# lnkloveating/MediQuery-RAG

Measured on AMD Instinct MI355X. Metric: queries/s (embed+top-k, k=5, b=256) over 1M×768 corpus; p50 single-query ms, higher is better.
Workload: dtype f32 (exact 3-way bf16 split, fp32 accumulate; exact fp32 top-k)

## Files before the change

mediquery-rag_amd/csrc/gemm_epi.hpp:

```cpp
#pragma once

#include "gemm_f32.hpp"
#include "gemm_x6p.hpp"

namespace mq {

enum Epi {
  EPI_BIAS = 0,
  EPI_GELU_ERF = 1,
  EPI_GELU_TANH = 2,
  EPI_RESID = 3,
  EPI_RESID_STATS = 4,
  EPI_RESID_LN_STATS = 5,
  EPI_BIAS_LNFOLD = 6,
  EPI_GELU_ERF_LNFOLD = 7,
  EPI_GELU_TANH_LNFOLD = 8
};
constexpr bool epi_is_lnfold(int epi) { return epi >= EPI_BIAS_LNFOLD && epi <= EPI_GELU_TANH_LNFOLD; }

__device__ __forceinline__ float gelu_erf(float x) {
  const float z = fabsf(x) * 0.70710678118654752f;
  const float t = __builtin_amdgcn_rcpf(fmaf(0.5f, z, 1.0f));
  float p = 0.17087277f;
  p = fmaf(p, t, -0.82215223f);
  p = fmaf(p, t, 1.48851587f);
  p = fmaf(p, t, -1.13520398f);
  p = fmaf(p, t, 0.27886807f);
  p = fmaf(p, t, -0.18628806f);
  p = fmaf(p, t, 0.09678418f);
  p = fmaf(p, t, 0.37409196f);
  p = fmaf(p, t, 1.00002368f);
  p = fmaf(p, t, -1.26551223f);
  const float e = t * __builtin_amdgcn_exp2f(fmaf(-z, z, p) * 1.4426950408889634f);
  return x * (x >= 0.f ? fmaf(-0.5f, e, 1.0f) : 0.5f * e);
}
__device__ __forceinline__ float gelu_tanh(float x) {
  const float u = 0.7978845608028654f * fmaf(0.044715f * x, x * x, x);
  return x * __builtin_amdgcn_rcpf(1.0f + __builtin_amdgcn_exp2f(u * -2.8853900817779268f));
}

template <int EPI>
__device__ __forceinline__ float epi_apply(float v) {
  if constexpr (EPI == EPI_GELU_ERF || EPI == EPI_GELU_ERF_LNFOLD) return gelu_erf(v);
  if constexpr (EPI == EPI_GELU_TANH || EPI == EPI_GELU_TANH_LNFOLD) return gelu_tanh(v);
  return v;
}

__device__ __forceinline__ void ln_merge(const floatx4 (&p)[kLnMaxParts / 2], float eps, float& mean, float& rstd) {
  float sum = 0.f;
#pragma unroll
  for (int i = 0; i < kLnMaxParts / 2; ++i) {
    sum += p[i].x;
    sum += p[i].z;
  }
  mean = sum * (1.0f / (float)kLnMaxParts);
  float m2 = 0.f;
#pragma unroll
  for (int i = 0; i < kLnMaxParts / 2; ++i) {
    const float d0 = p[i].x - mean, d1 = p[i].z - mean;
    m2 = __fmaf_rn((float)kLnPartW * d0, d0, m2 + p[i].y);
    m2 = __fmaf_rn((float)kLnPartW * d1, d1, m2 + p[i].w);
  }
  rstd = 1.0f / sqrtf(__fmaf_rn(m2, 1.0f / (float)(kLnPartW * kLnMaxParts), eps));
}
template <int MB>
__device__ __forceinline__ void ln_row_own(const float* __restrict__ stats, int wr0, int M, float eps, int lane,
                                           float& mean, float& rstd) {
  const int c = lane & 15;
  const int row = min(wr0 + 16 * min(c >> 2, MB - 1) + 4 * (lane >> 4) + (c & 3), M - 1);
  const floatx4* src = reinterpret_cast<const floatx4*>(stats + (int64_t)row * (2 * kLnMaxParts));
  floatx4 p[kLnMaxParts / 2];
#pragma unroll
  for (int i = 0; i < kLnMaxParts / 2; ++i) p[i] = src[i];
  ln_merge(p, eps, mean, rstd);
}
__device__ __forceinline__ float ln_row_bcast(float v, int lane, int m, int e) {
  return __shfl(v, (lane & 48) + 4 * m + e);
}
__device__ __forceinline__ float row16_sum(float v) {
  v += __int_as_float(__builtin_amdgcn_update_dpp(0, __float_as_int(v), 0xB1, 0xF, 0xF, false));
  v += __int_as_float(__builtin_amdgcn_update_dpp(0, __float_as_int(v), 0x4E, 0xF, 0xF, false));
  v += __int_as_float(__builtin_amdgcn_update_dpp(0, __float_as_int(v), 0x141, 0xF, 0xF, false));
  v += __int_as_float(__builtin_amdgcn_update_dpp(0, __float_as_int(v), 0x140, 0xF, 0xF, false));
  return v;
}

template <int EPI, int TM, int TN>
__device__ __forceinline__ void store_wave_tile(floatx16 (&acc)[TM][TN], int wr0, int wc0, int M, int N,
                                                const float* __restrict__ bias, const float* __restrict__ resid,
                                                int ldr, float* __restrict__ out, int ldo, int lane) {
  if (wr0 + TM * 32 <= M && wc0 + TN * 32 <= N) {
    float bv[TN];
#pragma unroll
    for (int tn = 0; tn < TN; ++tn) bv[tn] = bias[wc0 + tn * 32 + (lane & 31)];
    float rv[TM][TN][16];
    if constexpr (EPI == EPI_RESID) {
      const __amdgpu_buffer_rsrc_t rr = __builtin_amdgcn_make_buffer_rsrc(
          (void*)(resid + (int64_t)wr0 * ldr + wc0), (short)0, 0x7fffffff, 0x00020000);
      const int rl = (4 * (lane >> 5) * ldr + (lane & 31)) * 4;
#pragma unroll
      for (int tm = 0; tm < TM; ++tm)
#pragma unroll
        for (int tn = 0; tn < TN; ++tn)
#pragma unroll
          for (int e = 0; e < 16; ++e)
            rv[tm][tn][e] = __uint_as_float(
                __builtin_amdgcn_raw_buffer_load_b32(rr, rl, (acc_row(tm, e, 0) * ldr + tn * 32) * 4, 0));
    }
    const __amdgpu_buffer_rsrc_t ro = __builtin_amdgcn_make_buffer_rsrc(
        (void*)(out + (int64_t)wr0 * ldo + wc0), (short)0, 0x7fffffff, 0x00020000);
    const int ol = (4 * (lane >> 5) * ldo + (lane & 31)) * 4;
#pragma unroll
    for (int tm = 0; tm < TM; ++tm)
#pragma unroll
      for (int tn = 0; tn < TN; ++tn)
#pragma unroll
        for (int e = 0; e < 16; ++e) {
          float v = epi_apply<EPI>(acc[tm][tn][e] + bv[tn]);
          if constexpr (EPI == EPI_RESID) v += rv[tm][tn][e];
          __builtin_amdgcn_raw_buffer_store_b32(__float_as_uint(v), ro, ol, (acc_row(tm, e, 0) * ldo + tn * 32) * 4, 0);
        }
    return;
  }
#pragma unroll
  for (int tn = 0; tn < TN; ++tn) {
    const int col = wc0 + tn * 32 + (lane & 31);
    if (col >= N) continue;
    const float b = bias[col];
#pragma unroll
    for (int tm = 0; tm < TM; ++tm)
#pragma unroll
      for (int e = 0; e < 16; ++e) {
        const int row = wr0 + acc_row(tm, e, lane);
        if (row >= M) continue;
        float v = epi_apply<EPI>(acc[tm][tn][e] + b);
        if constexpr (EPI == EPI_RESID) v += resid[(int64_t)row * ldr + col];
        out[(int64_t)row * ldo + col] = v;
      }
  }
}

typedef unsigned uint2v_t __attribute__((ext_vector_type(2)));
template <int ER, int MB, int NB>
__device__ __forceinline__ void store_wave_tile16_ln_stats(floatx4 (&acc)[MB][NB], int wr0, int wc0, int M,
                                                           const float* __restrict__ bias,
                                                           const float* __restrict__ resid, int ldr,
                                                           float* __restrict__ out, int ldo, int lane,
                                                           const LnFold& lf) {
  static_assert(NB * 16 == kLnPartW && MB <= 4, "partials are per kLnPartW-column wave tile");
  const int c = lane & 15, g = lane >> 4;
  const bool ln_r = lf.stats_in != nullptr;
  float own_mu = 0.f, own_rho = 1.0f;
  if (ln_r) ln_row_own<MB>(lf.stats_in, wr0, M, lf.eps, lane, own_mu, own_rho);
  float gv[NB];
#pragma unroll
  for (int n = 0; n < NB; ++n) {
    const int col = wc0 + n * 16 + c;
    const float bb = bias[col] + (ln_r ? lf.b[col] : 0.f);
    gv[n] = ln_r ? lf.g[col] : 1.0f;
#pragma unroll
    for (int m = 0; m < MB; ++m)
#pragma unroll
      for (int e = 0; e < 4; ++e) acc[m][n][e] += bb;
  }
  const __amdgpu_buffer_rsrc_t rr =
      __builtin_amdgcn_make_buffer_rsrc((void*)(resid + wc0), (short)0, 0x7fffffff, 0x00020000);
  const __amdgpu_buffer_rsrc_t ro =
      __builtin_amdgcn_make_buffer_rsrc((void*)(out + wc0), (short)0, 0x7fffffff, 0x00020000);
  const __amdgpu_buffer_rsrc_t rs = __builtin_amdgcn_make_buffer_rsrc(
      (void*)(lf.stats_out + 2 * (wc0 / kLnPartW)), (short)0, 0x7fffffff, 0x00020000);
#pragma unroll
  for (int m = 0; m < MB; ++m)
#pragma unroll
    for (int eh = 0; eh < 4; eh += ER) {
      float v[ER][NB];
#pragma unroll
      for (int e2 = 0; e2 < ER; ++e2) {
        const int lo = (min(wr0 + m * 16 + 4 * g + eh + e2, M - 1) * ldr + c) * 4;
#pragma unroll
        for (int n = 0; n < NB; ++n)
          v[e2][n] = __uint_as_float(__builtin_amdgcn_raw_buffer_load_b32(rr, lo, n * 64, 0));
      }
#pragma unroll
      for (int e2 = 0; e2 < ER; ++e2) {
        const int e = eh + e2, row = wr0 + m * 16 + 4 * g + e;
        const float mu = ln_row_bcast(own_mu, lane, m, e), rho = ln_row_bcast(own_rho, lane, m, e);
        const int so = (row * ldo + c) * 4;
        float sum = 0.f;
#pragma unroll
        for (int n = 0; n < NB; ++n) {
          v[e2][n] = __fmaf_rn((v[e2][n] - mu) * rho, gv[n], acc[m][n][e]);
          sum += v[e2][n];
          if (row < M) __builtin_amdgcn_raw_buffer_store_b32(__float_as_uint(v[e2][n]), ro, so, n * 64, 0);
        }
        const float mean = row16_sum(sum) * (1.0f / (float)kLnPartW);
        float m2 = 0.f;
#pragma unroll
        for (int n = 0; n < NB; ++n) {
          const float d = v[e2][n] - mean;
          m2 = __fmaf_rn(d, d, m2);
        }
        m2 = row16_sum(m2);
        if (c == 0 && row < M) {
          uint2v_t pr;
          pr.x = __float_as_uint(mean);
          pr.y = __float_as_uint(m2);
          __builtin_amdgcn_raw_buffer_store_b64(pr, rs, row * (kLnMaxParts * 8), 0, 0);
        }
      }
    }
}

template <int EPI, int MB, int NB>
__device__ __forceinline__ void store_wave_tile16(floatx4 (&acc)[MB][NB], int wr0, int wc0, int M, int N,
                                                  const float* __restrict__ bias, const float* __restrict__ resid,
                                                  int ldr, float* __restrict__ out, int ldo, int lane,
                                                  const LnFold& lf = LnFold{}) {
  const int c = lane & 15, g = lane >> 4;
  if constexpr (EPI == EPI_RESID_LN_STATS) {
    store_wave_tile16_ln_stats<1>(acc, wr0, wc0, M, bias, resid, ldr, out, ldo, lane, lf);
    return;
  }
  constexpr bool FOLD = epi_is_lnfold(EPI);
  static_assert(!FOLD || MB <= 4, "one lane of a 16-lane row group per row of the wave tile");
  float own_mu = 0.f, own_rho = 0.f;
  if constexpr (FOLD) ln_row_own<MB>(lf.stats_in, wr0, M, lf.eps, lane, own_mu, own_rho);
  if (wr0 + MB * 16 <= M && wc0 + NB * 16 <= N) {
    float bv[NB], sv[NB];
#pragma unroll
    for (int n = 0; n < NB; ++n) bv[n] = bias[wc0 + n * 16 + c];
    if constexpr (FOLD) {
#pragma unroll
      for (int n = 0; n < NB; ++n) sv[n] = lf.s[wc0 + n * 16 + c];
    }
    const __amdgpu_buffer_rsrc_t rr = __builtin_amdgcn_make_buffer_rsrc(
        (void*)(resid + (EPI == EPI_RESID ? (int64_t)wr0 * ldr + wc0 : 0)), (short)0, 0x7fffffff, 0x00020000);
    const int rl = (4 * g * ldr + c) * 4;
    const __amdgpu_buffer_rsrc_t ro = __builtin_amdgcn_make_buffer_rsrc(
        (void*)(out + (int64_t)wr0 * ldo + wc0), (short)0, 0x7fffffff, 0x00020000);
    const int ol = (4 * g * ldo + c) * 4;
#pragma unroll
    for (int m = 0; m < MB; ++m) {
      float rv[NB][4];
      if constexpr (EPI == EPI_RESID) {
#pragma unroll
        for (int n = 0; n < NB; ++n)
#pragma unroll
          for (int e = 0; e < 4; ++e)
            rv[n][e] = __uint_as_float(
                __builtin_amdgcn_raw_buffer_load_b32(rr, rl, ((m * 16 + e) * ldr + n * 16) * 4, 0));
      }
      if constexpr (FOLD) {
#pragma unroll
        for (int e = 0; e < 4; ++e) {
          const float mu = ln_row_bcast(own_mu, lane, m, e), rho = ln_row_bcast(own_rho, lane, m, e);
#pragma unroll
          for (int n = 0; n < NB; ++n) {
            const float v = epi_apply<EPI>(__fmaf_rn(rho, __fmaf_rn(-mu, sv[n], acc[m][n][e]), bv[n]));
            __builtin_amdgcn_raw_buffer_store_b32(__float_as_uint(v), ro, ol, ((m * 16 + e) * ldo + n * 16) * 4, 0);
          }
        }
      } else {
#pragma unroll
        for (int n = 0; n < NB; ++n)
#pragma unroll
          for (int e = 0; e < 4; ++e) {
            float v = epi_apply<EPI>(acc[m][n][e] + bv[n]);
            if constexpr (EPI == EPI_RESID) v += rv[n][e];
            __builtin_amdgcn_raw_buffer_store_b32(__float_as_uint(v), ro, ol, ((m * 16 + e) * ldo + n * 16) * 4, 0);
          }
      }
    }
    return;
  }
  if constexpr (FOLD) {
#pragma unroll
    for (int m = 0; m < MB; ++m) {
      float mu[4], rho[4];
#pragma unroll
      for (int e = 0; e < 4; ++e) {
        mu[e] = ln_row_bcast(own_mu, lane, m, e);
        rho[e] = ln_row_bcast(own_rho, lane, m, e);
      }
#pragma unroll
      for (int n = 0; n < NB; ++n) {
        const int col = wc0 + n * 16 + c;
        if (col < N) {
          const float b = bias[col], sn = lf.s[col];
#pragma unroll
          for (int e = 0; e < 4; ++e) {
            const int row = wr0 + m * 16 + 4 * g + e;
            if (row < M)
              out[(int64_t)row * ldo + col] = epi_apply<EPI>(__fmaf_rn(rho[e], __fmaf_rn(-mu[e], sn, acc[m][n][e]), b));
          }
        }
      }
    }
    return;
  }
#pragma unroll
  for (int n = 0; n < NB; ++n) {
    const int col = wc0 + n * 16 + c;
    if (col >= N) continue;
    const float b = bias[col];
#pragma unroll
    for (int m = 0; m < MB; ++m)
#pragma unroll
      for (int e = 0; e < 4; ++e) {
        const int row = wr0 + m * 16 + 4 * g + e;
        if (row >= M) continue;
        float v = epi_apply<EPI>(acc[m][n][e] + b);
        if constexpr (EPI == EPI_RESID) v += resid[(int64_t)row * ldr + col];
        out[(int64_t)row * ldo + col] = v;
      }
  }
}

}
```

mediquery-rag_amd/csrc/gemm_x6p.hip:

```cpp
#include <algorithm>

#include "gemm_epi.hpp"
#include "gemm_x6p.hpp"

namespace mq {
namespace {

typedef __attribute__((address_space(3))) void x6p_lds_t;

__device__ __forceinline__ void x6p_glds(const void* base, unsigned voff, unsigned lds_dst) {
  const uint64_t b64 = (uint64_t)(uintptr_t)base;
  base = (const void*)(uintptr_t)(((uint64_t)__builtin_amdgcn_readfirstlane((unsigned)(b64 >> 32)) << 32) |
                                  (unsigned)__builtin_amdgcn_readfirstlane((unsigned)b64));
  unsigned keep;
  asm volatile("s_mov_b32 %0, m0\n\ts_mov_b32 m0, %3\n\ts_nop 0\n\tglobal_load_lds_dwordx4 %1, %2\n\ts_mov_b32 m0, %0"
               : "=&s"(keep)
               : "v"(voff), "s"(base), "s"(__builtin_amdgcn_readfirstlane(lds_dst))
               : "memory");
}

__device__ __forceinline__ int a_swz(int q) { return q ^ (q >> 1); }

typedef __bf16 bf16x2_t __attribute__((ext_vector_type(2)));
typedef float float2_t __attribute__((ext_vector_type(2)));
__device__ __forceinline__ unsigned cvt_pk_bf16(float lo, float hi) {
  float2_t v;
  v.x = lo;
  v.y = hi;
  return __builtin_bit_cast(unsigned, __builtin_convertvector(v, bf16x2_t));
}
__device__ __forceinline__ void split3v(floatx4 x, uint2 (&pl)[3]) {
#pragma unroll
  for (int p = 0; p < 3; ++p) {
    const unsigned a = cvt_pk_bf16(x.x, x.y), b = cvt_pk_bf16(x.z, x.w);
    pl[p] = make_uint2(a, b);
    if (p < 2) {
      x.x -= bf16_lo(a);
      x.y -= bf16_hi(a);
      x.z -= bf16_lo(b);
      x.w -= bf16_hi(b);
    }
  }
}

#if defined(MQ_X6P_DBG) && !defined(MQ_MEASUREMENT_BUILD)
#error "MQ_X6P_DBG computes wrong results: only a measurement build (-DMQ_MEASUREMENT_BUILD) may set it"
#endif

template <int WAVES_M_, int WAVES_N_, int TM_, int TN_, int NBUF_, int KS_ = 1, int DMAW_ = 8, bool SCHED_ = false,
          int DBG_ = 0, int DSTEP_ = 1, int BR0_ = 0, int PS_ = 4, bool LDR_ = false, bool M16_ = false,
          bool DEEP_ = false>
struct X6pTile {
  static constexpr int WAVES_M = WAVES_M_, WAVES_N = WAVES_N_, TM = TM_, TN = TN_, NBUF = NBUF_;
  static constexpr int KS = KS_;
  static constexpr int DMAW = DMAW_;
  static constexpr bool SCHED = SCHED_;
  static constexpr int DSTEP = DSTEP_, BR0 = BR0_, PS = PS_;
  static constexpr int DBG = DBG_;
  static constexpr bool LDR = LDR_;
  static constexpr bool M16 = M16_, DEEP = DEEP_;
  static constexpr int NW = WAVES_M * WAVES_N, THREADS = (LDR ? 2 * NW : NW) * 64;
  static constexpr int WM = TM * 32, WN = TN * 32, BM = WAVES_M * WM, BN = WAVES_N * WN;
  static constexpr int A_SUB = BM * 64;
  static constexpr int B_SUB = BN * 96;
  static constexpr int STAGE = KS * (A_SUB + B_SUB);
  static constexpr int NA = BM / 16, NB = BN / 32 * 3;
  static constexpr int NI = KS * (NA + NB);
  static constexpr int CNT_LO = NI / DMAW, REM = NI % DMAW, CNT_HI = CNT_LO + (REM ? 1 : 0);
  static_assert(DMAW == 8 || DMAW == 4, "DMA waves");
  static_assert(!LDR || DMAW == 4, "loader mode: the 4 loader waves issue every DMA");
  static constexpr int AHEAD = KS == 1 || (M16 && DEEP) ? NBUF : NBUF - 1;
  static_assert(!M16 || (KS == 2 && SCHED), "16x16x32 body: slot-scheduled 32-deep stages");
  static_assert(!DEEP || M16, "DEEP is a 16x16x32 option");
#ifndef MQ_X6P_GM
#define MQ_X6P_GM 4
#endif
  static constexpr int GM = MQ_X6P_GM;
  static_assert(LDR ? NW == 4 : NW == 8, "8-wave workgroups");
  static_assert(!SCHED || (CNT_HI - 1) * DSTEP < TM * TN * 6 * (M16 ? 4 : 1), "DMAs per k-step slots");
  static_assert(AHEAD >= 2 && NBUF * STAGE <= 160 * 1024, "LDS ring");
};

template <class T, int EPI>
__global__ __launch_bounds__(T::THREADS, 1) void gemm_x6p_kernel(const float* __restrict__ A, int lda,
                                                             const unsigned char* __restrict__ W3,
                                                             const float* __restrict__ bias,
                                                             const float* __restrict__ resid, int ldr,
                                                             float* __restrict__ out, int ldo, int M, int N,
                                                             int K, int rx, LnFold lf) {
  __shared__ __attribute__((aligned(1024))) unsigned char lds[T::NBUF * T::STAGE];
  const unsigned lds0 = (unsigned)(uintptr_t)(x6p_lds_t*)lds;
  const int lane = threadIdx.x & 63;
  const int wave = __builtin_amdgcn_readfirstlane(threadIdx.x >> 6);
  const int cw = T::LDR ? wave % T::NW : wave;
  const int wm = cw / T::WAVES_N, wn = cw % T::WAVES_N;
  const int tiles_m = (M + T::BM - 1) / T::BM, tiles_n = (N + T::BN - 1) / T::BN;
  const int total = tiles_m * tiles_n;
  const int G = gridDim.x, per_xcd = G >> 3;
  const int xslot = (blockIdx.x & 7) * per_xcd + (blockIdx.x >> 3);
  int m_lo = 0, rm = tiles_m, n_lo = 0, rn = tiles_n, loc = xslot, wstep = G, rtiles = total;
  if (rx > 0) {
    const Region rg = region_of(rx, blockIdx.x & 7, tiles_m, tiles_n);
    m_lo = rg.m_lo;
    rm = rg.rm;
    n_lo = rg.n_lo;
    rn = rg.rn;
    loc = blockIdx.x >> 3;
    wstep = per_xcd;
    rtiles = rm * rn;
  }
  const int n_tiles = loc < rtiles ? (rtiles - loc + wstep - 1) / wstep : 0;
  if (n_tiles == 0) return;
  const int nk = K >> 4;
  const int nst = nk / T::KS;
  const int S = n_tiles * nst;
  const int nbw = (N + 31) >> 5;
  const int band_tiles = T::GM * rn;
  auto coords = [&](int i, int& m0, int& n0) {
    const int t = i * wstep + loc;
    const int band = t / band_tiles;
    const int gm = min(T::GM, rm - band * T::GM);
    const int w = t - band * band_tiles;
    const int tc = w / gm;
    m0 = (m_lo + band * T::GM + (w - tc * gm)) * T::BM;
    n0 = (n_lo + tc) * T::BN;
  };

  int is_j = 0, is_i = 0, is_kt = 0, is_m0, is_n0;
  coords(0, is_m0, is_n0);
  const unsigned a_chunk = (unsigned)(((lane & 3) ^ a_swz((lane >> 4) & 3)) * 16);
  auto issue_one = [&](int buf, int t) __attribute__((always_inline)) {
    if constexpr (T::DBG & 1) return;
    if constexpr (T::DBG & 64) {
      if (is_j >= T::AHEAD) return;
    }
    const int dw = T::LDR ? wave - T::NW : wave;
    if (dw < 0 || dw >= T::DMAW || (T::REM && t == T::CNT_HI - 1 && dw >= T::REM)) return;
    const unsigned dst = lds0 + (unsigned)(buf * T::STAGE);
    const int ins = dw + t * T::DMAW;
    const int ks = ins / (T::NA + T::NB), in = ins - ks * (T::NA + T::NB);
    const int kt = is_kt + ks;
    if (in < T::NA) {
      if constexpr (T::DBG & 16) return;
      const float* abase = A + (int64_t)is_m0 * lda + kt * 16;
      const unsigned voff = (unsigned)min(16 * in + (lane >> 2), M - 1 - is_m0) * (unsigned)lda * 4u + a_chunk;
      x6p_glds(abase, voff, dst + ks * T::A_SUB + in * 1024);
    } else {
      if constexpr (T::DBG & 32) return;
      const int b = in - T::NA, nbl = b / 3, p = b - nbl * 3;
      const int nbg = min((is_n0 >> 5) + nbl, nbw - 1);
      const unsigned char* wbase = W3 + ((size_t)(nbg * nk + kt) * 3 + p) * 1024;
      x6p_glds(wbase, (unsigned)lane * 16u, dst + T::KS * T::A_SUB + ks * T::B_SUB + b * 1024);
    }
  };
  auto advance = [&]() __attribute__((always_inline)) {
    if (is_j + 1 < S) {
      ++is_j;
      is_kt += T::KS;
      if (is_kt == nk) {
        is_kt = 0;
        ++is_i;
        coords(is_i, is_m0, is_n0);
      }
    }
  };
  auto issue = [&](int buf) __attribute__((always_inline)) {
#pragma unroll
    for (int t = 0; t < T::CNT_HI; ++t) issue_one(buf, t);
    advance();
  };

  const int r = lane & 31, h = lane >> 5, sw = a_swz((r >> 2) & 3);
  const unsigned a_lo = (unsigned)((((2 * h) ^ sw) * 16)), a_hi = (unsigned)((((2 * h + 1) ^ sw) * 16));
  struct Frags {
    floatx4 raw[T::TM][2];
    bf16x8 a[T::TM][3], b[T::TN][3];
  };
  auto read_frags = [&](int buf, int ks, Frags& f) __attribute__((always_inline)) {
    if constexpr (T::DBG & 8) return;
    const unsigned char* st = lds + buf * T::STAGE;
#pragma unroll
    for (int tm = 0; tm < T::TM; ++tm) {
      const unsigned char* ar = st + ks * T::A_SUB + (wm * T::WM + tm * 32 + r) * 64;
      f.raw[tm][0] = *reinterpret_cast<const floatx4*>(ar + a_lo);
      f.raw[tm][1] = *reinterpret_cast<const floatx4*>(ar + a_hi);
    }
    const unsigned char* bs = st + T::KS * T::A_SUB + ks * T::B_SUB + lane * 16;
#pragma unroll
    for (int tn = 0; tn < T::TN; ++tn)
#pragma unroll
      for (int p = 0; p < 3; ++p)
        f.b[tn][p] = __builtin_bit_cast(bf16x8, *reinterpret_cast<const uintx4*>(bs + ((wn * T::TN + tn) * 3 + p) * 1024));
  };
  auto split_frags = [&](Frags& f) __attribute__((always_inline)) {
#pragma unroll
    for (int tm = 0; tm < T::TM; ++tm) {
      if constexpr (T::DBG & 2) {
        f.a[tm][0] = __builtin_bit_cast(bf16x8, f.raw[tm][0]);
        f.a[tm][1] = __builtin_bit_cast(bf16x8, f.raw[tm][1]);
        f.a[tm][2] = f.a[tm][0];
        continue;
      }
      uint2 pl[3], ph[3];
      split3v(f.raw[tm][0], pl);
      split3v(f.raw[tm][1], ph);
#pragma unroll
      for (int p = 0; p < 3; ++p) {
        uintx4 v;
        v.x = pl[p].x;
        v.y = pl[p].y;
        v.z = ph[p].x;
        v.w = ph[p].y;
        f.a[tm][p] = __builtin_bit_cast(bf16x8, v);
      }
    }
  };
  floatx16 acc[T::TM][T::TN];
  auto mma = [&](const Frags& f, auto&& hook) __attribute__((always_inline)) {
#pragma unroll
    for (int tm = 0; tm < T::TM; ++tm)
#pragma unroll
      for (int tn = 0; tn < T::TN; ++tn) {
        acc[tm][tn] = __builtin_amdgcn_mfma_f32_32x32x16_bf16(f.a[tm][2], f.b[tn][0], acc[tm][tn], 0, 0, 0);
        acc[tm][tn] = __builtin_amdgcn_mfma_f32_32x32x16_bf16(f.a[tm][1], f.b[tn][1], acc[tm][tn], 0, 0, 0);
        acc[tm][tn] = __builtin_amdgcn_mfma_f32_32x32x16_bf16(f.a[tm][0], f.b[tn][2], acc[tm][tn], 0, 0, 0);
        acc[tm][tn] = __builtin_amdgcn_mfma_f32_32x32x16_bf16(f.a[tm][1], f.b[tn][0], acc[tm][tn], 0, 0, 0);
        acc[tm][tn] = __builtin_amdgcn_mfma_f32_32x32x16_bf16(f.a[tm][0], f.b[tn][1], acc[tm][tn], 0, 0, 0);
        acc[tm][tn] = __builtin_amdgcn_mfma_f32_32x32x16_bf16(f.a[tm][0], f.b[tn][0], acc[tm][tn], 0, 0, 0);
        hook(tm * T::TN + tn);
      }
  };
  auto mma_one = [&](const Frags& f, int i) __attribute__((always_inline)) {
    const int g = i / 6, tm = g / T::TN, tn = g % T::TN, term = i % 6;
    const int pa = term == 0 ? 2 : term == 1 || term == 3 ? 1 : 0;
    const int pb = term == 0 || term >= 3 ? (term == 4 ? 1 : 0) : term == 1 ? 1 : 2;
    acc[tm][tn] = __builtin_amdgcn_mfma_f32_32x32x16_bf16(f.a[tm][pa], f.b[tn][pb], acc[tm][tn], 0, 0, 0);
  };
  auto read_a = [&](int buf, int ks, Frags& f) __attribute__((always_inline)) {
    if constexpr ((T::DBG & 8) || (T::DBG & 512)) {
#pragma unroll
      for (int tm = 0; tm < T::TM; ++tm) asm volatile("" : "+v"(f.raw[tm][0]), "+v"(f.raw[tm][1]));
      return;
    }
    const unsigned char* st = lds + buf * T::STAGE;
#pragma unroll
    for (int tm = 0; tm < T::TM; ++tm) {
      const unsigned char* ar = st + ks * T::A_SUB + (wm * T::WM + tm * 32 + r) * 64;
      f.raw[tm][0] = *reinterpret_cast<const floatx4*>(ar + a_lo);
      f.raw[tm][1] = *reinterpret_cast<const floatx4*>(ar + a_hi);
    }
  };
  auto read_b = [&](int buf, int ks, Frags& f, int q) __attribute__((always_inline)) {
    if constexpr ((T::DBG & 8) || (T::DBG & 256)) {
      asm volatile("" : "+v"(f.b[q / 3][q % 3]));
      return;
    }
    const unsigned char* bs = lds + buf * T::STAGE + T::KS * T::A_SUB + ks * T::B_SUB + lane * 16;
    f.b[q / 3][q % 3] = __builtin_bit_cast(bf16x8, *reinterpret_cast<const uintx4*>(bs + ((wn * T::TN) * 3 + q) * 1024));
  };
  unsigned pk[T::TM][2][3][2];
  auto piece = [&](Frags& f, int q) __attribute__((always_inline)) {
    const int tm = q / 12, half = (q / 6) % 2, p = (q % 6) / 2, part = q % 2;
    floatx4& x = f.raw[tm][half];
    unsigned u;
    if (part == 0) {
      u = cvt_pk_bf16(x.x, x.y);
      if (p < 2) {
        x.x -= bf16_lo(u);
        x.y -= bf16_hi(u);
      }
    } else {
      u = cvt_pk_bf16(x.z, x.w);
      if (p < 2) {
        x.z -= bf16_lo(u);
        x.w -= bf16_hi(u);
      }
    }
    asm volatile("" : "+v"(u), "+v"(x));
    pk[tm][half][p][part] = u;
  };
  auto assemble = [&](Frags& f) __attribute__((always_inline)) {
#pragma unroll
    for (int tm = 0; tm < T::TM; ++tm)
#pragma unroll
      for (int p = 0; p < 3; ++p) {
        uintx4 v;
        v.x = pk[tm][0][p][0];
        v.y = pk[tm][0][p][1];
        v.z = pk[tm][1][p][0];
        v.w = pk[tm][1][p][1];
        f.a[tm][p] = __builtin_bit_cast(bf16x8, v);
        asm volatile("" : "+v"(f.a[tm][p]));
      }
  };
  int c_i = 0, c_st = 0;
  auto tile_end = [&]() __attribute__((always_inline)) {
    if (++c_st == nst) {
      c_st = 0;
      int m0, n0;
      coords(c_i, m0, n0);
      if constexpr (!(T::DBG & 4))
        store_wave_tile<EPI, T::TM, T::TN>(acc, m0 + wm * T::WM, n0 + wn * T::WN, M, N, bias, resid, ldr, out, ldo,
                                           lane);
      zero_acc<T>(acc);
      ++c_i;
    }
  };
  auto wait_stages = [&](auto stages) __attribute__((always_inline)) {
    constexpr int n = decltype(stages)::value;
    const int dwi = T::LDR ? wave - T::NW : wave;
    if constexpr (T::DBG & 128) {
      if (T::REM && dwi >= 0 && dwi < T::REM)
        asm volatile("s_waitcnt vmcnt(%0)\n\ts_waitcnt lgkmcnt(0)" ::"n"(T::CNT_HI * n) : "memory");
      else
        asm volatile("s_waitcnt vmcnt(%0)\n\ts_waitcnt lgkmcnt(0)" ::"n"(T::CNT_LO * n) : "memory");
      return;
    }
    if (T::REM && dwi >= 0 && dwi < T::REM)
      asm volatile("s_waitcnt vmcnt(%0)" ::"n"(T::CNT_HI * n) : "memory");
    else
      asm volatile("s_waitcnt vmcnt(%0)" ::"n"(T::CNT_LO * n) : "memory");
    __builtin_amdgcn_s_waitcnt(0xC07F);
    asm volatile("s_barrier" ::: "memory");
  };
  zero_acc<T>(acc);

  if constexpr (T::LDR) {
    if (wave >= T::NW) {
#pragma unroll
      for (int d = 0; d < T::AHEAD; ++d) issue(d);
      wait_stages(IC<T::AHEAD - 1>{});
      for (int j = 0; j < S; ++j) {
        wait_stages(IC<T::AHEAD - 2>{});
        issue((j + T::AHEAD) % T::NBUF);
      }
      asm volatile("s_waitcnt vmcnt(0)" ::: "memory");
      return;
    }
  } else {
#pragma unroll
    for (int d = 0; d < T::AHEAD; ++d) issue(d);
  }
  if constexpr (T::M16) {
    constexpr int MB = 2 * T::TM, NB16 = 2 * T::TN, RS = NB16 * 6, NM16 = MB * RS, NSUB = 28;
    static_assert(RS >= NSUB + 4, "a region holds one block's split and its raw reads");
    const int c = lane & 15, kq = lane >> 4, hq = kq & 1, sw16 = a_swz((c >> 2) & 3);
    const unsigned a_base = (unsigned)((kq >> 1) * T::A_SUB + (wm * T::WM + c) * 64);
    const unsigned a_lo16 = a_base + (unsigned)(((2 * hq) ^ sw16) * 16);
    const unsigned a_hi16 = a_base + (unsigned)(((2 * hq + 1) ^ sw16) * 16);
    const unsigned b_base =
        (unsigned)(T::KS * T::A_SUB + (kq >> 1) * T::B_SUB + wn * T::TN * 3 * 1024 + hq * 512 + c * 16);
    floatx4 acc4[MB][NB16];
    uintx4 au[MB][3];
    bf16x8 bw[NB16][3];
    floatx4 raw[2];
    auto rd_raw = [&](const unsigned char* st, int m, int half) __attribute__((always_inline)) {
      raw[half] = *reinterpret_cast<const floatx4*>(st + m * 1024 + (half ? a_hi16 : a_lo16));
    };
    auto rd_b = [&](const unsigned char* st, int n, int p) __attribute__((always_inline)) {
      bw[n][p] = __builtin_bit_cast(
          bf16x8, *reinterpret_cast<const uintx4*>(st + b_base + ((n >> 1) * 3 + p) * 1024 + (n & 1) * 256));
    };
    auto sub = [&](int m, int q) __attribute__((always_inline)) {
      const int half = q / 14, rq = q % 14;
      const int p = rq < 12 ? rq / 6 : 2, part = rq < 12 ? (rq % 6) / 3 : rq - 12, op = rq < 12 ? rq % 3 : 0;
      floatx4& x = raw[half];
      if (op == 0) {
        unsigned u = cvt_pk_bf16(x[2 * part], x[2 * part + 1]);
        asm volatile("" : "+v"(u));
        au[m][p][2 * half + part] = u;
      } else {
        const unsigned u = au[m][p][2 * half + part];
        if (op == 1)
          x[2 * part] -= bf16_lo(u);
        else
          x[2 * part + 1] -= bf16_hi(u);
        asm volatile("" : "+v"(x));
      }
    };
    auto zero4 = [&]() __attribute__((always_inline)) {
#pragma unroll
      for (int m = 0; m < MB; ++m)
#pragma unroll
        for (int n = 0; n < NB16; ++n) acc4[m][n] = floatx4{0.f, 0.f, 0.f, 0.f};
    };
    zero4();
    wait_stages(IC<T::AHEAD - 1>{});
#pragma unroll
    for (int m = 0; m < MB; ++m) {
      rd_raw(lds, m, 0);
      rd_raw(lds, m, 1);
      if (m < MB - 1) {
#pragma unroll
        for (int q = 0; q < NSUB; ++q) sub(m, q);
      }
    }
#pragma unroll
    for (int n = 0; n < NB16; ++n)
#pragma unroll
      for (int p = 0; p < 3; ++p) rd_b(lds, n, p);
    int rb = 1 % T::NBUF;
    int ib = T::AHEAD % T::NBUF;
    for (int j = 0; j < S; ++j) {
      if constexpr (!T::LDR) {
        wait_stages(IC<T::AHEAD - 2>{});
      } else {
        if constexpr (T::DEEP) __builtin_amdgcn_s_waitcnt(0xC07F);
        asm volatile("s_barrier" ::: "memory");
      }
      const unsigned char* st = lds + rb * T::STAGE;
      static_for<NM16>([&](auto ic) {
        constexpr int i = decltype(ic)::value;
        constexpr int m = i / RS, w = i % RS, n = w / 6, term = w % 6;
        constexpr int pa = term == 0 ? 2 : term == 1 || term == 3 ? 1 : 0;
        constexpr int pb = term == 0 || term >= 3 ? (term == 4 ? 1 : 0) : term == 1 ? 1 : 2;
        acc4[m][n] = __builtin_amdgcn_mfma_f32_16x16x32_bf16(__builtin_bit_cast(bf16x8, au[m][pa]), bw[n][pb],
                                                             acc4[m][n], 0, 0, 0);
        if constexpr (w >= 2 && w < 2 + NSUB) sub((m + MB - 1) % MB, w - 2);
        if constexpr (w == 2 + NSUB || w == 3 + NSUB) rd_raw(st, m, w - 2 - NSUB);
        if constexpr (m == MB - 1 && term == 2) rd_b(st, n, 2);
        if constexpr (m == MB - 1 && term == 4) rd_b(st, n, 1);
        if constexpr (m == MB - 1 && term == 5) rd_b(st, n, 0);
        if constexpr (!T::LDR && i % T::DSTEP == 0 && i / T::DSTEP < T::CNT_HI) issue_one(ib, i / T::DSTEP);
        __builtin_amdgcn_sched_barrier(0);
      });
      if constexpr (!T::LDR) {
        advance();
        ib = ib + 1 == T::NBUF ? 0 : ib + 1;
      }
      rb = rb + 1 == T::NBUF ? 0 : rb + 1;
      if (++c_st == nst) {
        c_st = 0;
        int m0, n0;
        coords(c_i, m0, n0);
        store_wave_tile16<EPI, MB, NB16>(acc4, m0 + wm * T::WM, n0 + wn * T::WN, M, N, bias, resid, ldr, out, ldo,
                                         lane, lf);
        zero4();
        ++c_i;
      }
    }
    if constexpr (!T::LDR) asm volatile("s_waitcnt vmcnt(0)" ::: "memory");
    return;
  }
  wait_stages(IC<T::AHEAD - 1>{});
  Frags f0 = {}, f1 = {};
  read_frags(0, 0, f0);
  split_frags(f0);
  auto step = [&](int j, Frags& fa, Frags& fb) __attribute__((always_inline)) {
    wait_stages(IC<T::AHEAD - 2>{});
    const int buf = (j + T::AHEAD) % T::NBUF;
    if constexpr (!T::SCHED && !T::LDR) issue(buf);
    static_for<T::KS>([&](auto kc) {
      constexpr int ks = decltype(kc)::value;
      Frags& cur = ks % 2 == 0 ? fa : fb;
      Frags& nxt = ks % 2 == 0 ? fb : fa;
      if constexpr (T::SCHED) {
        constexpr int NM = T::TM * T::TN * 6, NBR = 3 * T::TN, PS = T::PS, NP = 12 * T::TM;
        constexpr int PER = (NP + (NM - PS) - 1) / (NM - PS);
        const int rbuf = ks + 1 < T::KS ? j % T::NBUF : (j + 1) % T::NBUF;
        constexpr int rks = ks + 1 < T::KS ? ks + 1 : 0;
        read_a(rbuf, rks, nxt);
        __builtin_amdgcn_sched_barrier(0);
        static_for<NM>([&](auto ic) {
          constexpr int i = decltype(ic)::value;
          mma_one(cur, i);
          constexpr bool dma_slot = !T::LDR && ks == 0 && i % T::DSTEP == 0 && i / T::DSTEP < T::CNT_HI;
          constexpr int bslot = [] {
            int n = 0;
            for (int k = T::BR0; k < i; ++k)
              if (!(!T::LDR && ks == 0 && k % T::DSTEP == 0 && k / T::DSTEP < T::CNT_HI) || T::DSTEP == 1) ++n;
            return n;
          }();
          if constexpr (i >= T::BR0 && (!dma_slot || T::DSTEP == 1)) {
            if constexpr (2 * bslot < NBR) read_b(rbuf, rks, nxt, 2 * bslot);
            if constexpr (2 * bslot + 1 < NBR) read_b(rbuf, rks, nxt, 2 * bslot + 1);
          }
          if constexpr (dma_slot) issue_one(buf, i / T::DSTEP);
          if constexpr (i >= PS) {
            static_for<PER>([&](auto pc) {
              constexpr int q = (i - PS) * PER + decltype(pc)::value;
              if constexpr (q < NP) piece(nxt, q);
            });
          }
          __builtin_amdgcn_sched_barrier(0);
        });
        assemble(nxt);
      } else {
        if constexpr (ks + 1 < T::KS)
          read_frags(j % T::NBUF, ks + 1, nxt);
        else
          read_frags((j + 1) % T::NBUF, 0, nxt);
        mma(cur, [](int) {});
        split_frags(nxt);
      }
    });
    if constexpr (T::SCHED && !T::LDR) advance();
    tile_end();
  };
  if constexpr (T::KS % 2 == 0) {
    for (int j = 0; j < S; ++j) step(j, f0, f1);
  } else {
    for (int j = 0; j < S; j += 2) {
      step(j, f0, f1);
      if (j + 1 >= S) break;
      step(j + 1, f1, f0);
    }
  }
  asm volatile("s_waitcnt vmcnt(0)" ::: "memory");
}

__global__ __launch_bounds__(256) void split_w3_kernel(const float* __restrict__ W, int N, int K,
                                                       uintx4* __restrict__ w3) {
  const int k8n = K >> 3, np = (N + 31) & ~31;
  const int64_t idx = (int64_t)blockIdx.x * 256 + threadIdx.x;
  if (idx >= (int64_t)np * k8n) return;
  const int n = (int)(idx / k8n), k8 = (int)(idx - (int64_t)n * k8n);
  floatx4 lo = {0.f, 0.f, 0.f, 0.f}, hi = lo;
  if (n < N) {
    lo = *reinterpret_cast<const floatx4*>(W + (int64_t)n * K + 8 * k8);
    hi = *reinterpret_cast<const floatx4*>(W + (int64_t)n * K + 8 * k8 + 4);
  }
  uint2 pl[3], ph[3];
  split3(lo, pl);
  split3(hi, ph);
  const int kb = k8 >> 1, hh = k8 & 1, nb = n >> 5, rr = n & 31;
#pragma unroll
  for (int p = 0; p < 3; ++p) {
    uintx4 v;
    v.x = pl[p].x;
    v.y = pl[p].y;
    v.z = ph[p].x;
    v.w = ph[p].y;
    w3[((int64_t)(nb * (K >> 4) + kb) * 3 + p) * 64 + hh * 32 + rr] = v;
  }
}

using X6p0 = X6pTile<2, 2, 2, 3, 3, 2, 4, true, 0, 1, 0, 6, true, true>;
using X6p1 = X6pTile<4, 1, 2, 3, 3, 2, 4, true, 0, 1, 0, 6, true, true>;
using X6p2 = X6pTile<4, 2, 1, 3, 3, 2, 4, true, 0, 2, 1, 6, false, true>;
using X6p3 = X6pTile<4, 2, 2, 3, 2, 2, 8, true, 0, 6, 1, 8, false, true, true>;
using X6p4 = X6pTile<2, 2, 2, 3, 3, 2, 4, true, 0, 1, 0, 6, true, true, true>;
using X6p5 = X6pTile<2, 2, 1, 3, 3, 2, 4, true, 0, 1, 0, 6, true, true, true>;
using X6p6 = X6pTile<4, 1, 2, 3, 3, 2, 4, true, 0, 1, 0, 6, true, true, true>;
using X6p7 = X6pTile<2, 2, 1, 3, 3, 2, 4, true, 0, 1, 0, 6, true, true>;
using X6p16 = X6pTile<2, 2, 2, 3, 4, 1, 4, true, 0, 1, 0, 6, true>;
using X6p17 = X6pTile<2, 2, 1, 3, 4, 1, 4, true, 0, 1, 0, 6, true>;

template <class T, int EPI>
void launch_t(const X6pArgs& g, int num_cus, hipStream_t s) {
  if constexpr (EPI < EPI_RESID_LN_STATS) {
    if (g.K % (16 * T::KS) != 0) {
      launch_t<X6pTile<4, 2, 1, 3, 4>, EPI>(g, num_cus, s);
      return;
    }
  }
  const int tiles = ((g.M + T::BM - 1) / T::BM) * ((g.N + T::BN - 1) / T::BN);
  const int grid = (std::min(tiles, num_cus) + 7) / 8 * 8;
  const int tiles_m = (g.M + T::BM - 1) / T::BM, tiles_n = (g.N + T::BN - 1) / T::BN;
  int rx = g.rx;
  if (rx < 0) rx = region_pick_rx(tiles_m, tiles_n, (double)T::BM * g.K * 4, (double)T::BN * g.K * 6, grid);
  if (rx > 0 && (8 % rx != 0 || rx > tiles_n || 8 / rx > tiles_m || grid < 8)) rx = 0;
  hipLaunchKernelGGL((gemm_x6p_kernel<T, EPI>), dim3(grid), dim3(T::THREADS), 0, s, g.A, g.lda,
                     static_cast<const unsigned char*>(g.W3), g.bias, g.resid, g.ldr, g.out, g.ldo, g.M, g.N, g.K, rx,
                     g.lf);
}

template <int EPI>
void launch_tile(const X6pArgs& g, int tile, int num_cus, hipStream_t s) {
#ifdef MQ_X6P_DBG
  if (tile >= 8) {
    switch (tile) {
      case 8: launch_t<X6pTile<2, 2, 2, 3, 4, 1, 4, true, 64, 1, 0, 6, true>, EPI>(g, num_cus, s); return;
      case 9: launch_t<X6pTile<2, 2, 2, 3, 4, 1, 4, true, 66, 1, 0, 6, true>, EPI>(g, num_cus, s); return;
      case 10: launch_t<X6pTile<2, 2, 2, 3, 4, 1, 4, true, 8, 1, 0, 6, true>, EPI>(g, num_cus, s); return;
      case 11: launch_t<X6pTile<2, 2, 2, 3, 4, 1, 4, true, 74, 1, 0, 6, true>, EPI>(g, num_cus, s); return;
      case 12: launch_t<X6pTile<2, 2, 2, 3, 4, 1, 4, true, 2, 1, 0, 6, true>, EPI>(g, num_cus, s); return;
      case 13: launch_t<X6pTile<2, 2, 2, 3, 4, 1, 4, true, 256, 1, 0, 6, true>, EPI>(g, num_cus, s); return;
      case 14: launch_t<X6pTile<2, 2, 2, 3, 4, 1, 4, true, 512, 1, 0, 6, true>, EPI>(g, num_cus, s); return;
      default: launch_t<X6pTile<2, 2, 2, 3, 4, 1, 4, true, 128, 1, 0, 6, true>, EPI>(g, num_cus, s); return;
    }
  }
#endif
  switch (tile) {
    case 1: launch_t<X6p1, EPI>(g, num_cus, s); return;
    case 2: launch_t<X6p2, EPI>(g, num_cus, s); return;
    case 3: launch_t<X6p3, EPI>(g, num_cus, s); return;
    case 4: launch_t<X6p4, EPI>(g, num_cus, s); return;
    case 5: launch_t<X6p5, EPI>(g, num_cus, s); return;
    case 6: launch_t<X6p6, EPI>(g, num_cus, s); return;
    case 7: launch_t<X6p7, EPI>(g, num_cus, s); return;
    case 16: launch_t<X6p16, EPI>(g, num_cus, s); return;
    case 17: launch_t<X6p17, EPI>(g, num_cus, s); return;
    default: launch_t<X6p0, EPI>(g, num_cus, s); return;
  }
}

template <int EPI>
void launch_tile_fold(const X6pArgs& g, int tile, int num_cus, hipStream_t s) {
  if (tile == 1)
    launch_t<X6p1, EPI>(g, num_cus, s);
  else
    launch_t<X6p0, EPI>(g, num_cus, s);
}

__global__ __launch_bounds__(256) void ln_fold_weight_kernel(const float* __restrict__ W,
                                                             const float* __restrict__ bias,
                                                             const float* __restrict__ g,
                                                             const float* __restrict__ b, int N, int K,
                                                             float* __restrict__ Wg, float* __restrict__ s_out,
                                                             float* __restrict__ c_out) {
  const int lane = threadIdx.x & 63;
  const int n = blockIdx.x * 4 + (threadIdx.x >> 6);
  if (n >= N) return;
  double sg = 0.0, sb = 0.0;
  for (int k = lane; k < K; k += 64) {
    const float w = W[(int64_t)n * K + k];
    const float wg = g[k] * w;
    Wg[(int64_t)n * K + k] = wg;
    sg += (double)wg;
    sb += (double)b[k] * (double)w;
  }
#pragma unroll
  for (int off = 32; off > 0; off >>= 1) {
    sg += __shfl_xor(sg, off);
    sb += __shfl_xor(sb, off);
  }
  if (lane == 0) {
    s_out[n] = (float)sg;
    c_out[n] = (float)((double)bias[n] + sb);
  }
}

}

void launch_ln_fold_weight(const float* W, const float* bias, const float* g, const float* b, int N, int K, float* Wg,
                           float* s_out, float* c_out, hipStream_t s) {
  hipLaunchKernelGGL(ln_fold_weight_kernel, dim3((unsigned)((N + 3) / 4)), dim3(256), 0, s, W, bias, g, b, N, K, Wg,
                     s_out, c_out);
}

void launch_split_w3(const float* W, int N, int K, void* w3, hipStream_t s) {
  const int64_t n = (int64_t)((N + 31) & ~31) * (K >> 3);
  hipLaunchKernelGGL(split_w3_kernel, dim3((unsigned)((n + 255) / 256)), dim3(256), 0, s, W, N, K,
                     static_cast<uintx4*>(w3));
}

int x6p_pick_tile(int M, int N, int num_cus) {
  auto rounds = [&](int bm, int bn) {
    const int64_t tiles = (int64_t)((M + bm - 1) / bm) * ((N + bn - 1) / bn);
    return (tiles + num_cus - 1) / num_cus;
  };
  return rounds(256, 96) < rounds(128, 192) ? 1 : 0;
}

void launch_gemm_x6p(const X6pArgs& g, int epi, int tile, int num_cus, hipStream_t s) {
  if (tile < 0) {
    tile = x6p_pick_tile(g.M, g.N, num_cus);
  }
  switch (epi) {
    case EPI_GELU_ERF: launch_tile<EPI_GELU_ERF>(g, tile, num_cus, s); return;
    case EPI_GELU_TANH: launch_tile<EPI_GELU_TANH>(g, tile, num_cus, s); return;
    case EPI_RESID: launch_tile<EPI_RESID>(g, tile, num_cus, s); return;
    case EPI_RESID_LN_STATS: launch_tile_fold<EPI_RESID_LN_STATS>(g, tile, num_cus, s); return;
    case EPI_BIAS_LNFOLD: launch_tile_fold<EPI_BIAS_LNFOLD>(g, tile, num_cus, s); return;
    case EPI_GELU_ERF_LNFOLD: launch_tile_fold<EPI_GELU_ERF_LNFOLD>(g, tile, num_cus, s); return;
    case EPI_GELU_TANH_LNFOLD: launch_tile_fold<EPI_GELU_TANH_LNFOLD>(g, tile, num_cus, s); return;
    default: launch_tile<EPI_BIAS>(g, tile, num_cus, s); return;
  }
}

}

extern "C" {

int64_t mq_debug_w3_bytes(int N, int K) { return N > 0 && K > 0 && K % 16 == 0 ? (int64_t)mq::w3_bytes(N, K) : -1; }

int mq_debug_split_w3(const float* W, int N, int K, void* w3, void* stream) {
  using namespace mq;
  clear_error();
  MQ_CHECK_ARG(W && w3, "NULL buffer");
  MQ_CHECK_ARG(N > 0 && K > 0 && K % 16 == 0, "bad shape N=%d K=%d", N, K);
  launch_split_w3(W, N, K, w3, (hipStream_t)stream);
  MQ_HIP(hipGetLastError());
  return MQ_OK;
}

int mq_debug_gemm_x6p(const float* A, const void* W3, const float* bias, const float* resid, float* out, int M,
                      int N, int K, int epi, int tile, void* stream) {
  using namespace mq;
  clear_error();
  MQ_CHECK_ARG(A && W3 && bias && out && (epi != EPI_RESID || resid), "NULL buffer");
  MQ_CHECK_ARG(M > 0 && N > 0 && K > 0 && K % 32 == 0, "bad shape M=%d N=%d K=%d", M, N, K);
  const int rx = tile >= 100 ? tile / 100 - 1 : -1;
  if (tile >= 100) tile %= 100;
  MQ_CHECK_ARG(epi >= 0 && epi <= 3 && tile >= -1 && tile <= 17 && rx <= 8, "bad epi/tile");
  int dev = 0, cus = 256;
  (void)hipGetDevice(&dev);
  (void)hipDeviceGetAttribute(&cus, hipDeviceAttributeMultiprocessorCount, dev);
  X6pArgs g{A, K, W3, bias, resid, N, out, N, M, N, K};
  g.rx = rx;
  launch_gemm_x6p(g, epi, tile, cus, (hipStream_t)stream);
  MQ_HIP(hipGetLastError());
  return MQ_OK;
}

int mq_debug_ln_fold_weight(const float* W, const float* bias, const float* g, const float* b, int N, int K,
                            float* Wg, float* s_out, float* c_out, void* stream) {
  using namespace mq;
  clear_error();
  MQ_CHECK_ARG(W && bias && g && b && Wg && s_out && c_out, "NULL buffer");
  MQ_CHECK_ARG(N > 0 && K > 0, "bad shape N=%d K=%d", N, K);
  launch_ln_fold_weight(W, bias, g, b, N, K, Wg, s_out, c_out, (hipStream_t)stream);
  MQ_HIP(hipGetLastError());
  return MQ_OK;
}

int mq_debug_gemm_x6p_ln(const float* A, const void* W3, const float* bias, const float* resid, float* out, int M,
                         int N, int K, int epi, int tile, const float* stats_in, float* stats_out, const float* g,
                         const float* b, const float* s_fold, float eps, void* stream) {
  using namespace mq;
  clear_error();
  MQ_CHECK_ARG(A && W3 && bias && out, "NULL buffer");
  MQ_CHECK_ARG(M > 0 && N > 0 && K > 0 && K % 32 == 0, "bad shape M=%d N=%d K=%d", M, N, K);
  MQ_CHECK_ARG(tile >= -1 && tile <= 1, "the LayerNorm-fold epilogues run on tiles 0 and 1 (got %d)", tile);
  if (epi == EPI_RESID_LN_STATS) {
    MQ_CHECK_ARG(resid && stats_out && (!stats_in || (g && b)), "producer: NULL buffer");
    MQ_CHECK_ARG(N == kLnPartW * kLnMaxParts, "producer: N must be %d (got %d)", kLnPartW * kLnMaxParts, N);
    MQ_CHECK_ARG((int64_t)M * N < (1ll << 29), "producer: M * N must stay below 2^29 (32-bit byte offsets)");
  } else {
    MQ_CHECK_ARG(epi_is_lnfold(epi), "epi must be a LayerNorm-fold kind (got %d)", epi);
    MQ_CHECK_ARG(stats_in && s_fold, "consumer: NULL buffer");
    MQ_CHECK_ARG(K == kLnPartW * kLnMaxParts, "consumer: K must be %d (got %d)", kLnPartW * kLnMaxParts, K);
  }
  int dev = 0, cus = 256;
  (void)hipGetDevice(&dev);
  (void)hipDeviceGetAttribute(&cus, hipDeviceAttributeMultiprocessorCount, dev);
  X6pArgs a{A, K, W3, bias, resid, N, out, N, M, N, K};
  a.lf.stats_in = stats_in;
  a.lf.stats_out = stats_out;
  a.lf.g = g;
  a.lf.b = b;
  a.lf.s = s_fold;
  a.lf.eps = eps;
  launch_gemm_x6p(a, epi, tile, cus, (hipStream_t)stream);
  MQ_HIP(hipGetLastError());
  return MQ_OK;
}

}
```

Measured before the change: 37150.

## Hand off residual LayerNorm epilogue prep from loader waves via LDS ring

In the producer LN-stats epilogue on loader-mode 16x16x32 tiles, the DMA loader waves, once their last stages are issued, load the residual tile and the LN partial stats, normalize the residual, and write it into a free LDS ring slot. After a barrier the compute waves read the normalized values from LDS instead of issuing global residual loads and row broadcasts. This takes the residual loads and the normalization off the compute waves' critical path and overlaps them with the final k-steps. The cost is extra barriers and LDS traffic plus tighter layout constraints, and tiles 20/21 keep the former epilogue for comparison.

```diff
diff --git a/mediquery-rag_amd/csrc/gemm_epi.hpp b/mediquery-rag_amd/csrc/gemm_epi.hpp
--- a/mediquery-rag_amd/csrc/gemm_epi.hpp
+++ b/mediquery-rag_amd/csrc/gemm_epi.hpp
@@ -141,17 +141,21 @@
 }
 
 typedef unsigned uint2v_t __attribute__((ext_vector_type(2)));
-template <int ER, int MB, int NB>
+__device__ __forceinline__ unsigned ln_t_slot(int lane) { return 16u * (unsigned)(lane ^ (lane >> 4)); }
+template <int ER, int MB, int NB, bool HAND = false>
 __device__ __forceinline__ void store_wave_tile16_ln_stats(floatx4 (&acc)[MB][NB], int wr0, int wc0, int M,
                                                            const float* __restrict__ bias,
                                                            const float* __restrict__ resid, int ldr,
                                                            float* __restrict__ out, int ldo, int lane,
-                                                           const LnFold& lf) {
+                                                           const LnFold& lf, const unsigned char* tl = nullptr) {
   static_assert(NB * 16 == kLnPartW && MB <= 4, "partials are per kLnPartW-column wave tile");
+  static_assert(!HAND || ER == 1, "the hand-off form finishes a row at a time");
   const int c = lane & 15, g = lane >> 4;
   const bool ln_r = lf.stats_in != nullptr;
   float own_mu = 0.f, own_rho = 1.0f;
-  if (ln_r) ln_row_own<MB>(lf.stats_in, wr0, M, lf.eps, lane, own_mu, own_rho);
+  if constexpr (!HAND) {
+    if (ln_r) ln_row_own<MB>(lf.stats_in, wr0, M, lf.eps, lane, own_mu, own_rho);
+  }
   float gv[NB];
 #pragma unroll
   for (int n = 0; n < NB; ++n) {
@@ -170,26 +174,41 @@
   const __amdgpu_buffer_rsrc_t rs = __builtin_amdgcn_make_buffer_rsrc(
       (void*)(lf.stats_out + 2 * (wc0 / kLnPartW)), (short)0, 0x7fffffff, 0x00020000);
 #pragma unroll
-  for (int m = 0; m < MB; ++m)
+  for (int m = 0; m < MB; ++m) {
+    floatx4 tv[NB];
+    if constexpr (HAND) {
+#pragma unroll
+      for (int n = 0; n < NB; ++n)
+        tv[n] = *reinterpret_cast<const floatx4*>(tl + (m * NB + n) * 1024 + ln_t_slot(lane));
+    }
 #pragma unroll
     for (int eh = 0; eh < 4; eh += ER) {
       float v[ER][NB];
-#pragma unroll
-      for (int e2 = 0; e2 < ER; ++e2) {
-        const int lo = (min(wr0 + m * 16 + 4 * g + eh + e2, M - 1) * ldr + c) * 4;
-#pragma unroll
-        for (int n = 0; n < NB; ++n)
-          v[e2][n] = __uint_as_float(__builtin_amdgcn_raw_buffer_load_b32(rr, lo, n * 64, 0));
+      if constexpr (!HAND) {
+#pragma unroll
+        for (int e2 = 0; e2 < ER; ++e2) {
+          const int lo = (min(wr0 + m * 16 + 4 * g + eh + e2, M - 1) * ldr + c) * 4;
+#pragma unroll
+          for (int n = 0; n < NB; ++n)
+            v[e2][n] = __uint_as_float(__builtin_amdgcn_raw_buffer_load_b32(rr, lo, n * 64, 0));
+        }
       }
 #pragma unroll
       for (int e2 = 0; e2 < ER; ++e2) {
         const int e = eh + e2, row = wr0 + m * 16 + 4 * g + e;
-        const float mu = ln_row_bcast(own_mu, lane, m, e), rho = ln_row_bcast(own_rho, lane, m, e);
+        float mu = 0.f, rho = 1.0f;
+        if constexpr (!HAND) {
+          mu = ln_row_bcast(own_mu, lane, m, e);
+          rho = ln_row_bcast(own_rho, lane, m, e);
+        }
         const int so = (row * ldo + c) * 4;
         float sum = 0.f;
 #pragma unroll
         for (int n = 0; n < NB; ++n) {
-          v[e2][n] = __fmaf_rn((v[e2][n] - mu) * rho, gv[n], acc[m][n][e]);
+          if constexpr (HAND)
+            v[e2][n] = __fmaf_rn(tv[n][e], gv[n], acc[m][n][e]);
+          else
+            v[e2][n] = __fmaf_rn((v[e2][n] - mu) * rho, gv[n], acc[m][n][e]);
           sum += v[e2][n];
           if (row < M) __builtin_amdgcn_raw_buffer_store_b32(__float_as_uint(v[e2][n]), ro, so, n * 64, 0);
         }
@@ -209,6 +228,60 @@
         }
       }
     }
+  }
+}
+
+template <int MB, int NB>
+struct LnTileRegs {
+  floatx4 r[MB][NB];
+  floatx4 p[kLnMaxParts / 2];
+};
+template <int Q>
+__device__ __forceinline__ float quad_bcast(float v) {
+  return __int_as_float(__builtin_amdgcn_update_dpp(0, __float_as_int(v), Q * 0x55, 0xF, 0xF, false));
+}
+template <int MB, int NB>
+__device__ __forceinline__ void ln_tile_load(LnTileRegs<MB, NB>& q, const float* __restrict__ resid, int ldr,
+                                             int wr0, int wc0, int M, const LnFold& lf, int lane) {
+  const __amdgpu_buffer_rsrc_t rr =
+      __builtin_amdgcn_make_buffer_rsrc((void*)(resid + wc0), (short)0, 0x7fffffff, 0x00020000);
+#pragma unroll
+  for (int m = 0; m < MB; ++m) {
+    const int row = min(wr0 + m * 16 + (lane >> 2), M - 1);
+    const int lo = (row * ldr + 4 * (lane & 3)) * 4;
+#pragma unroll
+    for (int n = 0; n < NB; ++n)
+      q.r[m][n] = __builtin_bit_cast(floatx4, __builtin_amdgcn_raw_buffer_load_b128(rr, lo, n * 64, 0));
+  }
+  if (lf.stats_in != nullptr) {
+    const int row = min(wr0 + (lane & 3) * 16 + (lane >> 2), M - 1);
+    const floatx4* src = reinterpret_cast<const floatx4*>(lf.stats_in + (int64_t)row * (2 * kLnMaxParts));
+#pragma unroll
+    for (int i = 0; i < kLnMaxParts / 2; ++i) q.p[i] = src[i];
+  }
+}
+template <int MB, int NB>
+__device__ __forceinline__ void ln_tile_write(const LnTileRegs<MB, NB>& q, unsigned char* tl, const LnFold& lf,
+                                              int lane) {
+  static_assert(MB == 4, "a quad's lanes share out the block rows");
+  const int g = lane >> 4, e = (lane >> 2) & 3;
+  unsigned off[4];
+#pragma unroll
+  for (int i = 0; i < 4; ++i) off[i] = (unsigned)(256 * g + 16 * ((4 * (lane & 3) + i) ^ g) + 4 * e);
+  float own_mu = 0.f, own_rho = 1.0f;
+  if (lf.stats_in != nullptr) ln_merge(q.p, lf.eps, own_mu, own_rho);
+  const float mus[4] = {quad_bcast<0>(own_mu), quad_bcast<1>(own_mu), quad_bcast<2>(own_mu), quad_bcast<3>(own_mu)};
+  const float rhos[4] = {quad_bcast<0>(own_rho), quad_bcast<1>(own_rho), quad_bcast<2>(own_rho),
+                         quad_bcast<3>(own_rho)};
+#pragma unroll
+  for (int m = 0; m < MB; ++m) {
+    const float mu = mus[m], rho = rhos[m];
+#pragma unroll
+    for (int n = 0; n < NB; ++n)
+#pragma unroll
+      for (int i = 0; i < 4; ++i)
+        *reinterpret_cast<float*>(tl + (m * NB + n) * 1024 + off[i]) = (q.r[m][n][i] - mu) * rho;
+  }
 }
 
 template <int EPI, int MB, int NB>
diff --git a/mediquery-rag_amd/csrc/gemm_x6p.hip b/mediquery-rag_amd/csrc/gemm_x6p.hip
--- a/mediquery-rag_amd/csrc/gemm_x6p.hip
+++ b/mediquery-rag_amd/csrc/gemm_x6p.hip
@@ -81,7 +81,7 @@
   static_assert(AHEAD >= 2 && NBUF * STAGE <= 160 * 1024, "LDS ring");
 };
 
-template <class T, int EPI>
+template <class T, int EPI, bool FORMER = false>
 __global__ __launch_bounds__(T::THREADS, 1) void gemm_x6p_kernel(const float* __restrict__ A, int lda,
                                                              const unsigned char* __restrict__ W3,
                                                              const float* __restrict__ bias,
@@ -90,6 +90,9 @@
                                                              int K, int rx, LnFold lf) {
   __shared__ __attribute__((aligned(1024))) unsigned char lds[T::NBUF * T::STAGE];
   const unsigned lds0 = (unsigned)(uintptr_t)(x6p_lds_t*)lds;
+  constexpr bool HAND = EPI == EPI_RESID_LN_STATS && T::LDR && T::M16 && !T::DEEP && T::NBUF == 3 && !FORMER;
+  static_assert(!HAND || (T::NW == 4 && 2 * T::WM * T::WN * 4 <= T::STAGE && T::WN == kLnPartW && T::STAGE % 1024 == 0),
+                "hand-off: two wave tiles of t per ring slot");
   const int lane = threadIdx.x & 63;
   const int wave = __builtin_amdgcn_readfirstlane(threadIdx.x >> 6);
   const int cw = T::LDR ? wave % T::NW : wave;
@@ -330,6 +333,24 @@
 #pragma unroll
       for (int d = 0; d < T::AHEAD; ++d) issue(d);
       wait_stages(IC<T::AHEAD - 1>{});
+      if constexpr (HAND) {
+        static_assert(T::AHEAD == 2, "hand-off: the ring two stages ahead");
+        for (int j = 0; j + 2 < S; ++j) {
+          wait_stages(IC<0>{});
+          issue((j + 2) % T::NBUF);
+        }
+        if (S >= 2) wait_stages(IC<0>{});
+        int m0, n0;
+        coords(n_tiles - 1, m0, n0);
+        LnTileRegs<2 * T::TM, 2 * T::TN> q;
+        ln_tile_load(q, resid, ldr, m0 + wm * T::WM, n0 + wn * T::WN, M, lf, lane);
+        wait_stages(IC<0>{});
+        const int ts = (S + (cw >> 1)) % T::NBUF;
+        ln_tile_write(q, lds + ts * T::STAGE + (cw & 1) * (T::WM * T::WN * 4), lf, lane);
+        __builtin_amdgcn_s_waitcnt(0xC07F);
+        asm volatile("s_barrier" ::: "memory");
+        return;
+      }
       for (int j = 0; j < S; ++j) {
         wait_stages(IC<T::AHEAD - 2>{});
         issue((j + T::AHEAD) % T::NBUF);
@@ -430,6 +451,9 @@
       }
       rb = rb + 1 == T::NBUF ? 0 : rb + 1;
       if (++c_st == nst) {
+        if constexpr (HAND) {
+          if (j == S - 1) break;
+        }
         c_st = 0;
         int m0, n0;
         coords(c_i, m0, n0);
@@ -438,6 +462,16 @@
         zero4();
         ++c_i;
       }
+    }
+    if constexpr (HAND) {
+      asm volatile("s_barrier" ::: "memory");
+      int m0, n0;
+      coords(n_tiles - 1, m0, n0);
+      const int ts = (S + (cw >> 1)) % T::NBUF;
+      store_wave_tile16_ln_stats<1, MB, NB16, true>(acc4, m0 + wm * T::WM, n0 + wn * T::WN, M, bias, resid, ldr, out,
+                                                    ldo, lane, lf,
+                                                    lds + ts * T::STAGE + (cw & 1) * (T::WM * T::WN * 4));
+      return;
     }
     if constexpr (!T::LDR) asm volatile("s_waitcnt vmcnt(0)" ::: "memory");
     return;
@@ -546,7 +580,7 @@
 using X6p16 = X6pTile<2, 2, 2, 3, 4, 1, 4, true, 0, 1, 0, 6, true>;
 using X6p17 = X6pTile<2, 2, 1, 3, 4, 1, 4, true, 0, 1, 0, 6, true>;
 
-template <class T, int EPI>
+template <class T, int EPI, bool FORMER = false>
 void launch_t(const X6pArgs& g, int num_cus, hipStream_t s) {
   if constexpr (EPI < EPI_RESID_LN_STATS) {
     if (g.K % (16 * T::KS) != 0) {
@@ -560,7 +594,7 @@
   int rx = g.rx;
   if (rx < 0) rx = region_pick_rx(tiles_m, tiles_n, (double)T::BM * g.K * 4, (double)T::BN * g.K * 6, grid);
   if (rx > 0 && (8 % rx != 0 || rx > tiles_n || 8 / rx > tiles_m || grid < 8)) rx = 0;
-  hipLaunchKernelGGL((gemm_x6p_kernel<T, EPI>), dim3(grid), dim3(T::THREADS), 0, s, g.A, g.lda,
+  hipLaunchKernelGGL((gemm_x6p_kernel<T, EPI, FORMER>), dim3(grid), dim3(T::THREADS), 0, s, g.A, g.lda,
                      static_cast<const unsigned char*>(g.W3), g.bias, g.resid, g.ldr, g.out, g.ldo, g.M, g.N, g.K, rx,
                      g.lf);
 }
@@ -597,10 +631,13 @@
 
 template <int EPI>
 void launch_tile_fold(const X6pArgs& g, int tile, int num_cus, hipStream_t s) {
-  if (tile == 1)
-    launch_t<X6p1, EPI>(g, num_cus, s);
-  else
-    launch_t<X6p0, EPI>(g, num_cus, s);
+  constexpr bool HAS_FORMER = EPI == EPI_RESID_LN_STATS;
+  switch (tile) {
+    case 1: launch_t<X6p1, EPI>(g, num_cus, s); return;
+    case 20: launch_t<X6p0, EPI, HAS_FORMER>(g, num_cus, s); return;
+    case 21: launch_t<X6p1, EPI, HAS_FORMER>(g, num_cus, s); return;
+    default: launch_t<X6p0, EPI>(g, num_cus, s); return;
+  }
 }
 
 __global__ __launch_bounds__(256) void ln_fold_weight_kernel(const float* __restrict__ W,
@@ -722,7 +759,8 @@
   clear_error();
   MQ_CHECK_ARG(A && W3 && bias && out, "NULL buffer");
   MQ_CHECK_ARG(M > 0 && N > 0 && K > 0 && K % 32 == 0, "bad shape M=%d N=%d K=%d", M, N, K);
-  MQ_CHECK_ARG(tile >= -1 && tile <= 1, "the LayerNorm-fold epilogues run on tiles 0 and 1 (got %d)", tile);
+  MQ_CHECK_ARG((tile >= -1 && tile <= 1) || tile == 20 || tile == 21,
+               "the LayerNorm-fold epilogues run on tiles 0 and 1 (20 / 21: their former epilogues; got %d)", tile);
   if (epi == EPI_RESID_LN_STATS) {
     MQ_CHECK_ARG(resid && stats_out && (!stats_in || (g && b)), "producer: NULL buffer");
     MQ_CHECK_ARG(N == kLnPartW * kLnMaxParts, "producer: N must be %d (got %d)", kLnPartW * kLnMaxParts, N);
```

After: 37720 (median of 6 runs). 1.02x the previous value.
